# Jagnate/GTA_graph_tensor_acclelrator_for_general_GNN

Measured on AMD Instinct MI355X. Metric: edges/sec + achieved HBM GB/s, GAT aggregate on Reddit, 1/2/4/8 MI355X, higher is better.
Workload: dtype f32; 1 GPU; GAT layer-1 aggregate block [3,11,12] (scatter C -> applyedge MUL -> gather ADD); graph=reddit-shaped, N=232965, E=114615892, F=128, heads=8, parallelism=one GPU, whole graph, mode=single, grid=1x1, row_chunks=1, impl=blocked, blocks=20, world_size_seen=1

## Files before the change

### gta_graph_tensor_acclelrator_for_general_gnn_amd/csrc/gta_kernels.hip

```cpp
#include <hip/hip_runtime.h>
#include <hip/hip_bf16.h>

#include <algorithm>
#include <atomic>
#include <cmath>
#include <cstdint>
#include <map>
#include <mutex>
#include <string>
#include <utility>

#include "../../include/gta.h"

namespace {

thread_local std::string g_err;

int fail(int code, const std::string& msg) {
  g_err = msg;
  return code;
}

#define GTA_HIP(x)                                                                   \
  do {                                                                               \
// ... 1624 lines not shown
  const int lane = threadIdx.x & (kWave - 1);
  const int64_t row = static_cast<int64_t>(blockIdx.x) * kWavesPerBlock + wave_id_uniform();
  if (row >= n_rows) return;
  const int col = lane * VW;
  const bool empty = ri.row_ptr[row] == ri.row_ptr[row + 1];
  float acc[VW];
  seg_reduce_fold<VW>(slabs, ri, row, lane, FoldMax<false>{0u}, acc);
  Vec<VW> o;
#pragma unroll
  for (int q = 0; q < VW; ++q) o.v[q] = empty ? 0.f : red_flip(acc[q], sbit);
  o.store(y + row * ldy + col);
}

template <int VW>
__global__ void __launch_bounds__(kBlock)
k_seg_reduce_att(int64_t n_rows, const float* __restrict__ slabs, int H, int normalize, float* __restrict__ y,
                 int64_t ldy, float* __restrict__ sums, RowItems ri, int skip_single = 0, int sf_out = GTA_SF_NONE) {
  const int lane = threadIdx.x & (kWave - 1);
  const int64_t row = static_cast<int64_t>(blockIdx.x) * kWavesPerBlock + wave_id_uniform();
  if (row >= n_rows) return;
  if (skip_single && ri.row_ptr[row + 1] - ri.row_ptr[row] == 1) return;
  const int col = lane * VW;
  constexpr int F = kWave * VW;
  const int64_t lds = F + ((H + 3) & ~3);
  const int head = col / (F / H);
  float acc[VW];
#pragma unroll
  for (int q = 0; q < VW; ++q) acc[q] = 0.f;
  float sh = 0.f, sl = 0.f;
  const bool any = ri.row_ptr[row + 1] > ri.row_ptr[row];
  for_row_items<VW>(ri, row, lane, [&](int64_t i0, int64_t i1, int64_t i2, int64_t i3, int m) {
    const int64_t id[4] = {i0, i1, i2, i3};
    for (int u = 0; u < m; ++u) {
      Vec<VW> p;
      p.load(slabs + id[u] * lds + col);
#pragma unroll
      for (int q = 0; q < VW; ++q) acc[q] += p.v[q];
      const float* ss = slabs + id[u] * lds + F;
      sh += ss[head];
      if (lane < H) sl += ss[lane];
    }
  });
  Vec<VW> o;
#pragma unroll
  for (int q = 0; q < VW; ++q) o.v[q] = normalize ? (any ? acc[q] / sh : 0.f) : acc[q];
  if (sf_out != GTA_SF_NONE) {
#pragma unroll
    for (int q = 0; q < VW; ++q) o.v[q] = sf_apply(sf_out, o.v[q]);
  }
  o.store(y + row * ldy + col);
  if (sums != nullptr && lane < H) sums[row * H + lane] = sl;
}

struct BlockedView {
  int64_t* hdr;
  int32_t* perm;
  int32_t* seg;
  int32_t* bucket;
  int64_t* row_ptr;
  int32_t* cnt;
  int64_t* scan;
  int32_t* lhist;
  SegItem* items;
  int32_t* row_items;
  int32_t* item_slot;
  SegItem* items_tmp;
};

inline int64_t blocked_max_items(int64_t n_rows, int64_t nnz, int B, int64_t item_edges) {
  return std::min<int64_t>(n_rows * B, nnz) + nnz / item_edges;
}

constexpr int64_t kScanMaxTiles = 4096;

constexpr int kLenBins = 257;

inline int64_t blocked_fixed_bytes(int64_t n_rows, int B) {
  return round16(128) + round16(n_rows * 4) + round16(n_rows * (B + 1) * 4) + round16(64 * 4) +
         round16((n_rows + 1) * 8) + round16(n_rows * B * 4) + round16((kScanMaxTiles + 1) * 8) +
         round16(2 * 64 * kLenBins * 4);
}

BlockedView blocked_view(void* base, int64_t n_rows, int B, int64_t max_items) {
  char* p = static_cast<char*>(base);
  BlockedView v;
  v.hdr = reinterpret_cast<int64_t*>(p); p += round16(16 * 8);
  v.perm = reinterpret_cast<int32_t*>(p); p += round16(n_rows * 4);
  v.seg = reinterpret_cast<int32_t*>(p); p += round16(n_rows * (B + 1) * 4);
  v.bucket = reinterpret_cast<int32_t*>(p); p += round16(64 * 4);
  v.row_ptr = reinterpret_cast<int64_t*>(p); p += round16((n_rows + 1) * 8);
  v.cnt = reinterpret_cast<int32_t*>(p); p += round16(n_rows * B * 4);
  v.scan = reinterpret_cast<int64_t*>(p); p += round16((kScanMaxTiles + 1) * 8);
  v.lhist = reinterpret_cast<int32_t*>(p); p += round16(2 * 64 * kLenBins * 4);
  v.items = reinterpret_cast<SegItem*>(p); p += round16(max_items * 16);
  v.row_items = reinterpret_cast<int32_t*>(p); p += round16(max_items * 4);
  v.item_slot = reinterpret_cast<int32_t*>(p); p += round16(max_items * 4);
  v.items_tmp = reinterpret_cast<SegItem*>(p);
  return v;
}

int64_t blocked_bytes(int64_t n_rows, int B, int64_t max_items) {
  return blocked_fixed_bytes(n_rows, B) + round16(max_items * 16) + round16(max_items * 4) + round16(max_items * 4) +
         round16(max_items * 16);
}

__device__ __forceinline__ int deg_bucket(int64_t d) {
  return d <= 1 ? 0 : min(31, 63 - __clzll(static_cast<unsigned long long>(d)));
}

__host__ __device__ __forceinline__ int64_t n_parts(int64_t len, int64_t item_edges) {
  return (len + item_edges - 1) / item_edges;
}

__device__ __forceinline__ int merge_of(int64_t deg, int B, int64_t row_edges) {
  if (row_edges <= 0 || deg <= 0) return 1;
  int m = 1;
  while (m < B && deg * m < row_edges * B) m <<= 1;
  return m;
}

__global__ void __launch_bounds__(kBlock)
k_blocked_seg(const int64_t* __restrict__ indptr, const int32_t* __restrict__ indices, int64_t n_rows, int B,
              int64_t bsize, int64_t item_edges, int64_t row_edges, BlockedView v) {
  const int lane = threadIdx.x & (kWave - 1);
  const int64_t row = static_cast<int64_t>(blockIdx.x) * kWavesPerBlock + wave_id_uniform();
  if (row >= n_rows) return;
  const int64_t rb = indptr[row], re = indptr[row + 1];
  int64_t pos = 0;
  for (int b = lane; b <= B; b += kWave) {
    const int64_t key = static_cast<int64_t>(b) * bsize;
    int64_t lo = rb, hi = re;
    while (lo < hi) {
      const int64_t mid = (lo + hi) >> 1;
      if (static_cast<int64_t>(indices[mid]) < key) lo = mid + 1; else hi = mid;
    }
    pos = (b == B ? re : lo) - rb;
    v.seg[row * (B + 1) + b] = static_cast<int32_t>(pos);
  }
  const int m = merge_of(re - rb, B, row_edges);
  const int nb = (B + m - 1) / m;
  const int64_t lo = __shfl(pos, min(lane * m, B));
  const int64_t hi = __shfl(pos, min((lane + 1) * m, B));
  int64_t parts = (lane < nb) ? n_parts(hi - lo, item_edges) : 0;
#pragma unroll
  for (int off = 32; off > 0; off >>= 1) parts += __shfl_xor(parts, off);
  if (lane == 0) v.row_ptr[row] = parts;
  bool bad = false;
  for (int64_t e = rb + lane; e + 1 < re; e += kWave) bad |= indices[e] > indices[e + 1];
  if (__any(bad) && lane == 0) atomicOr(reinterpret_cast<unsigned long long*>(&v.hdr[3]), 1ull);
  if (lane == 0) atomicAdd(&v.bucket[deg_bucket(re - rb)], 1);
}

__global__ void k_blocked_scan(BlockedView v) {
  if (threadIdx.x == 0) {
    int run = 0;
    for (int k = 31; k >= 0; --k) {
      v.bucket[32 + k] = run;
      run += v.bucket[k];
    }
  }
}

__global__ void k_blocked_perm(const int64_t* __restrict__ indptr, int64_t n_rows, BlockedView v) {
  const int64_t r = static_cast<int64_t>(blockIdx.x) * blockDim.x + threadIdx.x;
  if (r >= n_rows) return;
  const int k = deg_bucket(indptr[r + 1] - indptr[r]);
  const int pos = atomicAdd(&v.bucket[32 + k], 1);
  v.perm[pos] = static_cast<int32_t>(r);
}

__global__ void k_blocked_cnt(int64_t n_rows, int B, int64_t item_edges, int64_t row_edges, BlockedView v) {
  const int64_t k = static_cast<int64_t>(blockIdx.x) * blockDim.x + threadIdx.x;
  if (k >= n_rows * B) return;
  const int b = static_cast<int>(k / n_rows);
  const int32_t row = v.perm[k - static_cast<int64_t>(b) * n_rows];
  const int32_t* sg = v.seg + static_cast<int64_t>(row) * (B + 1);
  const int m = merge_of(sg[B], B, row_edges);
  v.cnt[k] = (b % m) ? 0 : static_cast<int32_t>(n_parts(sg[min(b + m, B)] - sg[b], item_edges));
}

template <typename T>
__global__ void __launch_bounds__(1024) k_scan_excl(T* __restrict__ a, int64_t n, int total_at_end,
                                                    int64_t* __restrict__ total) {
  __shared__ int64_t part[1024];
  const int t = threadIdx.x;
  const int64_t per = (n + 1023) / 1024;
  const int64_t b = min<int64_t>(n, t * per), e = min<int64_t>(n, b + per);
  int64_t s = 0;
  for (int64_t i = b; i < e; ++i) s += a[i];
  part[t] = s;
  __syncthreads();
  for (int off = 1; off < 1024; off <<= 1) {
    const int64_t x = (t >= off) ? part[t - off] : 0;
    __syncthreads();
    part[t] += x;
    __syncthreads();
  }
  int64_t run = (t == 0) ? 0 : part[t - 1];
  for (int64_t i = b; i < e; ++i) {
    const int64_t x = a[i];
    a[i] = static_cast<T>(run);
    run += x;
  }
  if (t == 1023) {
    if (total_at_end) a[n] = static_cast<T>(part[1023]);
    if (total) *total = part[1023];
  }
}

constexpr int kScanPer = 16;
constexpr int64_t kScanTile = 1024 * kScanPer;

template <typename T>
__global__ void __launch_bounds__(1024) k_scan_tiles(const T* __restrict__ a, int64_t n, int64_t tile,
                                                     int64_t* __restrict__ sums) {
  __shared__ int64_t red[16];
  const int t = threadIdx.x;
  const int64_t b0 = static_cast<int64_t>(blockIdx.x) * tile, b1 = min<int64_t>(n, b0 + tile);
  int64_t s = 0;
  for (int64_t i = b0 + t; i < b1; i += 1024) s += a[i];
#pragma unroll
  for (int off = 32; off > 0; off >>= 1) s += __shfl_xor(s, off);
  if ((t & 63) == 0) red[t >> 6] = s;
  __syncthreads();
  if (t == 0) {
    int64_t tot = 0;
    for (int w = 0; w < 16; ++w) tot += red[w];
    sums[blockIdx.x] = tot;
  }
}

template <typename T>
__global__ void __launch_bounds__(1024) k_scan_apply(T* __restrict__ a, int64_t n, int64_t tile,
                                                     const int64_t* __restrict__ offs, int64_t nt, int total_at_end,
                                                     int64_t* __restrict__ total) {
  __shared__ int64_t part[1024];
  const int t = threadIdx.x;
  const int64_t b0 = static_cast<int64_t>(blockIdx.x) * tile, b1 = min<int64_t>(n, b0 + tile);
  const int64_t per = tile / 1024;
  const int64_t e0 = min<int64_t>(b1, b0 + t * per), e1 = min<int64_t>(b1, e0 + per);
  int64_t s = 0;
  for (int64_t i = e0; i < e1; ++i) s += a[i];
  part[t] = s;
  __syncthreads();
  for (int off = 1; off < 1024; off <<= 1) {
    const int64_t x = (t >= off) ? part[t - off] : 0;
    __syncthreads();
    part[t] += x;
    __syncthreads();
  }
  int64_t run = offs[blockIdx.x] + ((t == 0) ? 0 : part[t - 1]);
  for (int64_t i = e0; i < e1; ++i) {
    const int64_t x = a[i];
    a[i] = static_cast<T>(run);
    run += x;
  }
  if (blockIdx.x == nt - 1 && t == 0) {
    if (total_at_end) a[n] = static_cast<T>(offs[nt]);
    if (total) *total = offs[nt];
  }
}

template <typename T>
void scan_excl(T* a, int64_t n, int total_at_end, int64_t* total, int64_t* scratch, hipStream_t s) {
  int64_t tile = kScanTile;
  while ((n + tile - 1) / tile > kScanMaxTiles) tile *= 2;
  const int64_t nt = (n + tile - 1) / tile;
  if (nt <= 1) {
    k_scan_excl<T><<<1, 1024, 0, s>>>(a, n, total_at_end, total);
    return;
  }
  k_scan_tiles<T><<<dim3(static_cast<unsigned>(nt)), dim3(1024), 0, s>>>(a, n, tile, scratch);
  k_scan_excl<int64_t><<<1, 1024, 0, s>>>(scratch, nt, 1, nullptr);
  k_scan_apply<T><<<dim3(static_cast<unsigned>(nt)), dim3(1024), 0, s>>>(a, n, tile, scratch, nt, total_at_end, total);
}

__global__ void k_blocked_items(const int64_t* __restrict__ indptr, int64_t n_rows, int B, int64_t item_edges,
                                int64_t row_edges, BlockedView v) {
  const int64_t k = static_cast<int64_t>(blockIdx.x) * blockDim.x + threadIdx.x;
  if (k >= n_rows * B) return;
  const int b = static_cast<int>(k / n_rows);
  const int32_t row = v.perm[k - static_cast<int64_t>(b) * n_rows];
  const int32_t* sg = v.seg + static_cast<int64_t>(row) * (B + 1);
  const int m = merge_of(sg[B], B, row_edges);
  if (b % m) return;
  const int64_t len = sg[min(b + m, B)] - sg[b];
  if (len == 0) return;
  int64_t before = 0;
  for (int q = 0; q < b; q += m) before += n_parts(sg[min(q + m, B)] - sg[q], item_edges);
  const int64_t parts = n_parts(len, item_edges), part = (len + parts - 1) / parts;
  const int64_t id0 = v.cnt[k], slot0 = v.row_ptr[row] + before, beg = indptr[row] + sg[b];
  for (int64_t j = 0; j < parts; ++j) {
    SegItem it;
    it.beg = beg + j * part;
    it.row = row;
    it.len = static_cast<int32_t>(max<int64_t>(0, min<int64_t>(part, len - j * part)));
    v.items[id0 + j] = it;
    v.row_items[slot0 + j] = static_cast<int32_t>(id0 + j);
    v.item_slot[id0 + j] = static_cast<int32_t>(slot0 + j);
    atomicAdd(&v.lhist[b * kLenBins + 256 - min(it.len, 256)], 1);
  }
}

__device__ __forceinline__ int len_key(int len) { return 256 - min(len, 256); }

__global__ void k_items_len_scan(BlockedView v, int64_t n_rows, int B) {
  const int b = threadIdx.x;
  if (b >= B) return;
  int run = v.cnt[static_cast<int64_t>(b) * n_rows];
  for (int key = 0; key < kLenBins; ++key) {
    const int c = v.lhist[b * kLenBins + key];
    v.lhist[64 * kLenBins + b * kLenBins + key] = run;
    run += c;
  }
}

__global__ void k_items_permute(BlockedView v, int64_t n_rows, int B) {
  const int64_t id = static_cast<int64_t>(blockIdx.x) * blockDim.x + threadIdx.x;
  if (id >= v.hdr[4]) return;
  int lo = 0, hi = B - 1;
  while (lo < hi) {
    const int mid = (lo + hi + 1) >> 1;
    if (v.cnt[static_cast<int64_t>(mid) * n_rows] <= id) lo = mid; else hi = mid - 1;
  }
  const SegItem it = v.items[id];
  const int nid = atomicAdd(&v.lhist[64 * kLenBins + lo * kLenBins + len_key(it.len)], 1);
  v.items_tmp[nid] = it;
  v.row_items[v.item_slot[id]] = nid;
}

__global__ void __launch_bounds__(kBlock)
k_aggregate_combine(PlanView plan, int F, const float* __restrict__ row_scale, float* __restrict__ y, int64_t ldy,
                    int accumulate, const float* __restrict__ partial, const void* __restrict__ xs = nullptr,
                    int64_t ldxs = 0, int xs_bf16 = 0, const float* __restrict__ self_scale = nullptr,
                    int y_bf16 = 0) {
  const int lane = threadIdx.x & (kWave - 1);
  const int64_t s = static_cast<int64_t>(blockIdx.x) * kWavesPerBlock + wave_id_uniform();
  if (s >= plan.hdr[1]) return;
  const int64_t row = plan.split_row[s];
  const int64_t first = plan.split_first[s];
  const int cnt = plan.split_cnt[s];
  const float scale = row_scale ? row_scale[row] : 1.f;
  for (int c = lane; c < F; c += kWave) {
    float a = 0.f;
    for (int j = 0; j < cnt; ++j) a += partial[(first + j) * F + c];
    float* yp = y + row * ldy + c;
    float v;
    if (xs != nullptr) {
#pragma clang fp contract(off)
      const float xv = xs_bf16 ? load_elem(static_cast<const uint16_t*>(xs) + row * ldxs + c)
                               : static_cast<const float*>(xs)[row * ldxs + c];
      v = xv * (self_scale ? *self_scale : 1.f) + scale * a;
    } else {
      v = accumulate ? (*yp + scale * a) : scale * a;
    }
    if (y_bf16) reinterpret_cast<uint16_t*>(y)[row * ldy + c] = to_bf16_bits(v);
    else *yp = v;
  }
}

template <typename UNIT>
__global__ void __launch_bounds__(kBlock)
k_scatter(int dir, const int64_t* __restrict__ indptr, const int32_t* __restrict__ indices, int64_t n_rows,
          const UNIT* __restrict__ x, int64_t ldx_u, int64_t row_u, UNIT* __restrict__ out, int64_t ldo_u) {
  const int lane = threadIdx.x & (kWave - 1);
  const int64_t row = static_cast<int64_t>(blockIdx.x) * kWavesPerBlock + wave_id_uniform();
  if (row >= n_rows) return;
  const int64_t eb = indptr[row], ee = indptr[row + 1];
  const int64_t total = (ee - eb) * row_u;
  for (int64_t t = lane; t < total; t += kWave) {
    const int64_t el = t / row_u, c = t - el * row_u;
    const int64_t e = eb + el;
    const int64_t src = (dir == GTA_DIR_R) ? row : indices[e];
    out[e * ldo_u + c] = x[src * ldx_u + c];
  }
}

__device__ __forceinline__ int64_t edge_row(int mode, int64_t e, int64_t row, const int32_t* indices) {
  return mode == GTA_IDX_EDGE ? e : (mode == GTA_IDX_SRC ? static_cast<int64_t>(indices[e]) : row);
// ... 1799 lines not shown
bool dispatch_x(int xm, int wm, bool bf, const AggArgs& a, int64_t nb, hipStream_t s) {
  if (xm >= XM_EX1) return !bf && wm == WM_NONE && dispatch_expr<LPE, VW, NV>(xm, a, nb, s);
  return xm == XM_EDGE ? dispatch_w<LPE, VW, NV, XM_EDGE>(wm, bf, a, nb, s)
                       : dispatch_w<LPE, VW, NV, XM_IDX>(wm, bf, a, nb, s);
}

template <int LPE>
bool dispatch_bf16_vw8(int ur, int wm, const AggArgs& a, int64_t nb, hipStream_t s) {
  if (wm == WM_EDGE1) {
    if (ur == 8) launch_agg<LPE, 8, 1, XM_IDX, WM_EDGE1, uint16_t, 8>(a, nb, s);
    else launch_agg<LPE, 8, 1, XM_IDX, WM_EDGE1, uint16_t, 4>(a, nb, s);
  } else {
    if (ur == 8) launch_agg<LPE, 8, 1, XM_IDX, WM_NONE, uint16_t, 8>(a, nb, s);
    else launch_agg<LPE, 8, 1, XM_IDX, WM_NONE, uint16_t, 4>(a, nb, s);
  }
  return true;
}

template <int N>
using IC = std::integral_constant<int, N>;

template <int VW, class Fn>
bool dispatch_lpe(int lpe, int nv, Fn fn) {
  switch (lpe) {
    case 64:
      if constexpr (VW < 8) {
        if (nv == 2) return fn(IC<VW>{}, IC<64>{}, IC<2>{});
        if (nv != 1) return fn(IC<VW>{}, IC<64>{}, IC<4>{});
      }
      return fn(IC<VW>{}, IC<64>{}, IC<1>{});
    case 32: return fn(IC<VW>{}, IC<32>{}, IC<1>{});
    case 16: return fn(IC<VW>{}, IC<16>{}, IC<1>{});
    case 8: return fn(IC<VW>{}, IC<8>{}, IC<1>{});
    default: return fn(IC<VW>{}, IC<4>{}, IC<1>{});
  }
}

template <class Fn>
bool dispatch_vw(int vw, int lpe, int nv, Fn fn) {
  return vw == 4 ? dispatch_lpe<4>(lpe, nv, fn) : (vw == 2 ? dispatch_lpe<2>(lpe, nv, fn) : dispatch_lpe<1>(lpe, nv, fn));
}

struct Tuning {
  int force_lpe = 0;
  int force_vw = 0;
  int agg_lean = 1;
  int seg_lean = 1;
  int seg_lean_w1 = 1;
  int seg_pf = 0;
  int seg_alpha1 = 1;
  int agg_bf16_vw8 = 4;
  int agg_w1 = 1;
  int expr_lean = 1;
  int seg_phase = 0;
  int att_lean = 1;
  int att_direct = 1;
  int apply_node_vec = 1;
  int apply_edge_form = 1;
  int esm_lane = 1;
  int mm_ring = 1;
  int mm_ring_fr = 0;
  int mm_ring_depth = 0;
  int mm_prefetch = 1;
  int64_t mm_split = -1;
  int mm_wave = 1;
  int mm_wave_fr = 0;
};

Tuning& thread_tuning() {
  thread_local Tuning t;
  return t;
}

std::mutex g_attach_mu;
std::map<void*, Tuning> g_attached;
std::atomic<int> g_attached_n{0};
thread_local const Tuning* t_call = nullptr;

struct CallTuning {
  const Tuning* prev = t_call;
  Tuning snap;
  explicit CallTuning(void* stream) {
    if (g_attached_n.load(std::memory_order_acquire) == 0) return;
    std::lock_guard<std::mutex> lk(g_attach_mu);
    auto it = g_attached.find(stream);
    if (it == g_attached.end()) return;
    snap = it->second;
    t_call = &snap;
  }
  ~CallTuning() { t_call = prev; }
  CallTuning(const CallTuning&) = delete;
  CallTuning& operator=(const CallTuning&) = delete;
};

const Tuning& tuning() { return t_call ? *t_call : thread_tuning(); }

struct Knob {
  const char* key;
  int Tuning::*i32;
  int64_t Tuning::*i64;
};

const Knob* find_knob(const char* key) {
  static const Knob knobs[] = {
      {"agg_lpe", &Tuning::force_lpe, nullptr},
      {"agg_vw", &Tuning::force_vw, nullptr},
      {"agg_lean", &Tuning::agg_lean, nullptr},
      {"seg_lean", &Tuning::seg_lean, nullptr},
      {"seg_lean_w1", &Tuning::seg_lean_w1, nullptr},
      {"seg_alpha1", &Tuning::seg_alpha1, nullptr},
      {"seg_pf", &Tuning::seg_pf, nullptr},
      {"agg_bf16_vw8", &Tuning::agg_bf16_vw8, nullptr},
      {"agg_w1", &Tuning::agg_w1, nullptr},
      {"expr_lean", &Tuning::expr_lean, nullptr},
      {"seg_phase", &Tuning::seg_phase, nullptr},
      {"att_lean", &Tuning::att_lean, nullptr},
      {"att_direct", &Tuning::att_direct, nullptr},
      {"apply_node_vec", &Tuning::apply_node_vec, nullptr},
      {"apply_edge_form", &Tuning::apply_edge_form, nullptr},
      {"esm_lane", &Tuning::esm_lane, nullptr},
      {"mm_ring", &Tuning::mm_ring, nullptr},
      {"mm_ring_fr", &Tuning::mm_ring_fr, nullptr},
      {"mm_ring_depth", &Tuning::mm_ring_depth, nullptr},
      {"mm_prefetch", &Tuning::mm_prefetch, nullptr},
      {"mm_split", nullptr, &Tuning::mm_split},
      {"mm_wave", &Tuning::mm_wave, nullptr},
      {"mm_wave_fr", &Tuning::mm_wave_fr, nullptr},
  };
  const std::string k(key ? key : "");
  for (const Knob& kb : knobs)
    if (k == kb.key) return &kb;
  return nullptr;
}

}

extern "C" {

int gta_abi_version(void) { return GTA_ABI_VERSION; }
const char* gta_last_error(void) { return g_err.c_str(); }

int gta_debug_set(const char* key, int64_t value) {
  const Knob* kb = find_knob(key);
  if (!kb) return fail(GTA_ERR_ARG, std::string("gta_debug_set: unknown key ") + (key ? key : ""));
  if (kb->i32) thread_tuning().*(kb->i32) = static_cast<int>(value);
  else thread_tuning().*(kb->i64) = value;
  return GTA_OK;
}

int gta_debug_get(const char* key, int64_t* value) {
  const Knob* kb = find_knob(key);
  if (!kb || !value) return fail(GTA_ERR_ARG, std::string("gta_debug_get: unknown key ") + (key ? key : ""));
  *value = kb->i32 ? static_cast<int64_t>(thread_tuning().*(kb->i32)) : thread_tuning().*(kb->i64);
  return GTA_OK;
}

}

struct gta_tuning {
  Tuning t;
};

extern "C" {

gta_tuning* gta_tuning_create(void) { return new (std::nothrow) gta_tuning{}; }

void gta_tuning_destroy(gta_tuning* h) { delete h; }
// ... 384 lines not shown
    code |= (bins[i] << (8 + 3 * i)) | (sfs[i] << (17 + 4 * i));
  }
  const int nl = shape == 1 ? (bins[0] == GTA_BIN_NONE ? 1 : 2) : shape + 1;
  for (int l = 0; l < 4; ++l) {
    const int k = l < nl ? l : 0;
    if (modes[k] != GTA_IDX_EDGE && modes[k] != GTA_IDX_SRC && modes[k] != GTA_IDX_DST)
      return fail(GTA_ERR_ARG, "aggregate_expr: bad operand mode");
    if ((lds[k] < F && !(modes[k] == GTA_IDX_EDGE && lds[k] == 0)) || (nnz > 0 && !operands[k]))
      return fail(GTA_ERR_ARG, "aggregate_expr: operand rows need ld >= F (or ld 0: a broadcast row)");
    if (lds[k] > INT32_MAX) return fail(GTA_ERR_UNSUPPORTED, "aggregate_expr: operand row stride >= 2^31");
    ex.p[l] = operands[k];
    ex.ld[l] = static_cast<int>(lds[k]);
    code |= modes[k] << (2 * l);
  }
  ex.code = code;
  return aggregate_impl(indptr, indices, n_rows, nnz, GTA_IDX_EDGE, ex.p[0], F, F, GTA_F32, nullptr, 0, 0, nullptr,
                        y, ldy, 0, plan, plan_chunk, workspace, stream, nullptr, 0, nullptr, 0, &ex, XM_EX1 + shape - 1);
}

int gta_aggregate_self(const int64_t* indptr, const int32_t* indices, int64_t n_rows, int64_t nnz, int x_mode,
                       const void* x, int64_t ldx, int64_t F, int x_dtype, const float* w, int64_t ldw, int64_t heads,
                       const float* row_scale, const void* x_self, int64_t ld_self, const float* self_scale, void* y,
                       int64_t ldy, int y_dtype, const void* plan, int64_t plan_chunk, void* workspace, void* stream) {
  if (!x_self) return fail(GTA_ERR_ARG, "aggregate_self: x_self is NULL");
  if (y_dtype != GTA_F32 && y_dtype != GTA_BF16) return fail(GTA_ERR_ARG, "aggregate_self: y_dtype must be F32 or BF16");
  return aggregate_impl(indptr, indices, n_rows, nnz, x_mode, x, ldx, F, x_dtype, w, ldw, heads, row_scale,
                        static_cast<float*>(y), ldy, 0, plan, plan_chunk, workspace, stream, x_self, ld_self, self_scale,
                        y_dtype == GTA_BF16 ? 1 : 0);
}

int64_t gta_aggregate_blocked_plan_bytes(int64_t n_rows, int64_t nnz, int64_t blocks, int64_t item_edges) {
  if (n_rows < 0 || nnz < 0 || blocks < 1 || blocks > 63 || item_edges < 1)
    return fail(GTA_ERR_ARG, "blocked_plan_bytes: need n_rows, nnz >= 0, 1 <= blocks <= 63, item_edges >= 1");
  const int B = static_cast<int>(blocks);
  return blocked_bytes(n_rows, B, blocked_max_items(n_rows, nnz, B, item_edges));
}

int gta_aggregate_blocked_plan_build(const int64_t* indptr, const int32_t* indices, int64_t n_rows, int64_t n_cols,
                                     int64_t nnz, int64_t blocks, int64_t item_edges, int64_t row_edges, void* plan,
                                     int64_t plan_bytes, void* stream) {
  const CallTuning ct_(stream);
  if (!indptr || !plan || n_rows <= 0 || n_cols <= 0 || nnz < 0 || blocks < 1 || blocks > 63 || item_edges < 1 ||
      row_edges < 0)
    return fail(GTA_ERR_ARG, "blocked_plan_build: bad arguments");
  if (nnz > 0 && !indices) return fail(GTA_ERR_ARG, "blocked_plan_build: indices needed");
  if (n_rows > INT32_MAX) return fail(GTA_ERR_UNSUPPORTED, "blocked_plan_build: > 2^31 rows");
  const int B = static_cast<int>(blocks);
  const int64_t mi = blocked_max_items(n_rows, nnz, B, item_edges);
  if (mi > INT32_MAX || n_rows * B > INT32_MAX) return fail(GTA_ERR_UNSUPPORTED, "blocked_plan_build: > 2^31 items");
  if (plan_bytes < blocked_bytes(n_rows, B, mi)) return fail(GTA_ERR_ARG, "blocked_plan_build: plan buffer too small");
  BlockedView v = blocked_view(plan, n_rows, B, mi);
  hipStream_t s = S(stream);
  const int64_t bsize = (n_cols + B - 1) / B;
  const int64_t hdr[16] = {B, bsize, n_rows, 0, 0, item_edges, mi,
                           reinterpret_cast<char*>(v.row_items) - static_cast<char*>(plan), row_edges};
  GTA_HIP(hipMemcpyAsync(v.hdr, hdr, sizeof(hdr), hipMemcpyHostToDevice, s));
  GTA_HIP(hipMemsetAsync(v.bucket, 0, 64 * 4, s));
  k_blocked_seg<<<dim3(static_cast<unsigned>((n_rows + kWavesPerBlock - 1) / kWavesPerBlock)), dim3(kBlock), 0, s>>>(
      indptr, indices, n_rows, B, bsize, item_edges, row_edges, v);
  GTA_LAUNCHED("k_blocked_seg");
  k_blocked_scan<<<1, 64, 0, s>>>(v);
  GTA_LAUNCHED("k_blocked_scan");
  k_blocked_perm<<<dim3(static_cast<unsigned>((n_rows + 255) / 256)), dim3(256), 0, s>>>(indptr, n_rows, v);
  GTA_LAUNCHED("k_blocked_perm");
  scan_excl<int64_t>(v.row_ptr, n_rows, 1, nullptr, v.scan, s);
  GTA_LAUNCHED("scan_excl");
  const dim3 gk(static_cast<unsigned>((n_rows * B + 255) / 256));
  k_blocked_cnt<<<gk, dim3(256), 0, s>>>(n_rows, B, item_edges, row_edges, v);
  GTA_LAUNCHED("k_blocked_cnt");
  scan_excl<int32_t>(v.cnt, n_rows * B, 0, &v.hdr[4], v.scan, s);
  GTA_LAUNCHED("scan_excl");
  GTA_HIP(hipMemsetAsync(v.lhist, 0, 64 * kLenBins * 4, s));
  k_blocked_items<<<gk, dim3(256), 0, s>>>(indptr, n_rows, B, item_edges, row_edges, v);
  GTA_LAUNCHED("k_blocked_items");
  if (mi > 0) {
    k_items_len_scan<<<1, 64, 0, s>>>(v, n_rows, B);
    GTA_LAUNCHED("k_items_len_scan");
    k_items_permute<<<dim3(static_cast<unsigned>((mi + 255) / 256)), dim3(256), 0, s>>>(v, n_rows, B);
    GTA_LAUNCHED("k_items_permute");
    GTA_HIP(hipMemcpyAsync(v.items, v.items_tmp, mi * sizeof(SegItem), hipMemcpyDeviceToDevice, s));
  }
  return GTA_OK;
}


int64_t gta_aggregate_blocked_workspace_bytes(int64_t n_rows, int64_t nnz, int64_t blocks, int64_t F,
                                              int64_t item_edges) {
  if (n_rows < 0 || nnz < 0 || blocks < 1 || blocks > 63 || F <= 0 || item_edges < 1)
    return fail(GTA_ERR_ARG, "blocked_workspace_bytes: bad sizes");
  return blocked_max_items(n_rows, nnz, static_cast<int>(blocks), item_edges) * F * static_cast<int64_t>(sizeof(float));
}

static int aggregate_blocked_impl(const std::string& who, const int64_t* indptr, const int32_t* indices, int64_t n_rows,
                                  int64_t n_cols, int64_t nnz, const void* xv, int64_t ldx, int64_t F, int x_dtype,
                                  const float* w, int64_t ldw, int64_t heads, const float* row_scale, float* y,
                                  int64_t ldy, int accumulate, const void* plan, int64_t blocks, int64_t item_edges,
                                  void* workspace, void* stream) {
  const CallTuning ct_(stream);
  if (n_rows < 0 || nnz < 0 || F <= 0 || blocks < 1 || blocks > 63 || item_edges < 1)
    return fail(GTA_ERR_ARG, who + ": bad sizes");
  if (x_dtype != GTA_F32 && x_dtype != GTA_BF16) return fail(GTA_ERR_ARG, who + ": x_dtype must be F32 or BF16");
  if (n_rows == 0) return GTA_OK;
  if (!indptr || !xv || !y || !plan) return fail(GTA_ERR_ARG, who + ": bad arguments");
  const bool bf = x_dtype == GTA_BF16;
  const float* x = static_cast<const float*>(xv);
  int gl = 0, vw = 0;
  for (int c : {4, 2, 1}) {
    if (F == static_cast<int64_t>(kWave) * c && (bf || (ldx % c == 0 && aligned(x, 4 * c))) && ldy % c == 0 &&
        aligned(y, 4 * c)) {
      vw = c;
      break;
    }
  }
  if (!vw) return fail(GTA_ERR_UNSUPPORTED, who + ": F must be 64, 128 or 256 (one edge per wave row)");
  bool gl_ok = true;
  if (w) {
    if (heads <= 0 || F % heads) return fail(GTA_ERR_ARG, who + ": heads must divide F");
    gl = static_cast<int>(F / heads) / vw;
    gl_ok = (F / heads) % vw == 0 && (gl == 4 || gl == 8 || gl == 16);
  }
  const std::string gl_msg = who + ": (F/heads)/VW must be 4, 8 or 16 (or quarter-wave lanes per head 1..16)";
  const BlockedCall c(plan, n_rows, nnz, blocks, item_edges, workspace, stream);
  if (!workspace && nnz > 0) return fail(GTA_ERR_ARG, who + ": needs the slab workspace");
  const int vq = static_cast<int>(F / 16);
  const int lph = w ? static_cast<int>((F / heads) / vq) : 0;
  const bool quarter = (vq == 4 || vq == 8 || vq == 16) && ldx % (bf ? 8 : 4) == 0 && aligned(x, 16) &&
                       (!w || ((F / heads) % vq == 0 && lph >= 1 && 16 % lph == 0));
  if (bf && !quarter)
    return fail(GTA_ERR_UNSUPPORTED, who + ": bf16 rows need x 16-B aligned, ldx % 8 == 0 and heads that fit the "
                                           "multi-item forms (F/heads a multiple of F/16, lanes per head dividing 16)");
  const int phase = tuning().seg_phase;
// ... 1068 lines not shown
```

### gta_graph_tensor_acclelrator_for_general_gnn_amd/graph.py

```python
import math

import torch

SHAPES = {
    "cora": (2708, 10556),
    "citeseer": (3327, 9228),
    "pubmed": (19717, 88648),
    "flickr": (89250, 899756),
    "reddit": (232965, 114615892),
    "products": (2449029, 123718280),
}


class Graph:

    def __init__(self, indptr, indices, n_cols=None):
        if indptr.dtype != torch.int64 or indices.dtype != torch.int32:
            raise TypeError("indptr must be int64 and indices int32")
        if indptr.device != indices.device:
            raise ValueError("indptr and indices on different devices")
        self.indptr = indptr.contiguous()
        self.indices = indices.contiguous()
        self.n_rows = indptr.numel() - 1
        self.n_cols = self.n_rows if n_cols is None else int(n_cols)
        self.nnz = indices.numel()
        self._plans = {}
        self._row_of_edge = None
        self._deg = None

    @property
    def device(self):
        return self.indptr.device

    def to(self, device):
        return Graph(self.indptr.to(device), self.indices.to(device), self.n_cols)

    def degrees(self):
        if self._deg is None:
            self._deg = (self.indptr[1:] - self.indptr[:-1])
        return self._deg

    def row_of_edge(self):
        if self._row_of_edge is None:
            rows = torch.arange(self.n_rows, device=self.device, dtype=torch.int32)
            self._row_of_edge = torch.repeat_interleave(rows, self.degrees())
        return self._row_of_edge

    def csc(self):
        if "csc" not in self._plans:
            from . import ops
            self._plans["csc"] = ops.CSC(self)
        return self._plans["csc"]

    def plan(self, chunk=512):
        if chunk not in self._plans:
            from . import ops
            self._plans[chunk] = ops.AggregatePlan(self, chunk)
        return self._plans[chunk]

    def blocked_plan(self, blocks=32, item_edges=None, row_edges=None):
        from . import ops
        key = ("blocked", blocks, int(item_edges or ops.BlockedPlan.ITEM_EDGES),
               int(ops.BlockedPlan.ROW_EDGES if row_edges is None else row_edges))
        if key not in self._plans:
            self._plans[key] = ops.BlockedPlan(self, blocks, key[2], key[3])
        return self._plans[key]

    def numpy(self):
        return self.indptr.cpu().numpy(), self.indices.cpu().numpy()

    def __repr__(self):
        return f"Graph(N={self.n_rows}, E={self.nnz}, device={self.device})"


def from_numpy(indptr, indices, device="cpu", n_cols=None):
    return Graph(torch.as_tensor(indptr, dtype=torch.int64).to(device),
                 torch.as_tensor(indices, dtype=torch.int32).to(device), n_cols)


def lognormal_degrees(n, e, seed=0, sigma=1.0, device="cpu"):
    g = torch.Generator(device=device)
    g.manual_seed(seed)
    z = torch.randn(n, generator=g, device=device, dtype=torch.float64)
    raw = torch.exp(sigma * z)
    scaled = raw * (e / raw.sum())
    deg = torch.floor(scaled).to(torch.int64)
    rem = int(e - int(deg.sum().item()))
    if rem > 0:
        frac = scaled - deg.to(torch.float64)
        top = torch.topk(frac, rem).indices
        deg[top] += 1
    return deg


def synthetic(n, e, seed=0, kind="lognormal", sigma=1.0, device="cpu", sort_cols=True, dedupe=False,
              locality_width=None):
    device = torch.device(device)
    if kind == "uniform":
        deg = torch.full((n,), e // n, dtype=torch.int64, device=device)
        deg[: e - int(deg.sum())] += 1
    elif kind == "lognormal":
        deg = lognormal_degrees(n, e, seed=seed, sigma=sigma, device=device)
    else:
        raise ValueError(kind)
    g = torch.Generator(device=device)
    g.manual_seed(seed + 1)
    rows = torch.repeat_interleave(torch.arange(n, device=device, dtype=torch.int64), deg)
    if locality_width is None:
        cols = torch.randint(0, n, (e,), generator=g, device=device, dtype=torch.int64)
    else:
        off = torch.randint(-locality_width, locality_width + 1, (e,), generator=g, device=device,
                            dtype=torch.int64)
        cols = torch.remainder(rows + off, n)
    if dedupe:
        keep = cols != rows
        rows, cols = rows[keep], cols[keep]
    if sort_cols or dedupe:
        key = rows * n + cols
# ... 115 lines not shown
```

### gta_graph_tensor_acclelrator_for_general_gnn_amd/ops.py

```python
import ctypes
import math
import threading
import weakref

import torch

from . import _lib
from ._lib import check

_MODES = {"edge": _lib.IDX_EDGE, "src": _lib.IDX_SRC, "dst": _lib.IDX_DST}
_BINS = {None: _lib.BIN_NONE, "NONE": _lib.BIN_NONE, "ADD": _lib.BIN_ADD, "MUL": _lib.BIN_MUL,
         "DIV": _lib.BIN_DIV, "SUB": _lib.BIN_SUB}


def _L():
    return _lib.load()


def _stream(dev):
    return torch.cuda.current_stream(dev).cuda_stream


def _need_gpu(*ts):
    for t in ts:
# ... 191 lines not shown
                          _ptr(x), ldx, F, x_dt, _ptr(out), ldy, _ptr(pbuf), chunk, _ptr(ws), _stream(x.device)),
          "reduce")
    return out


EXPR_SHAPES = {1: 2, 2: 3, 3: 4}


def aggregate_expr(graph, shape, operands, bins, sfs=None, swap=False, plan=None):
    if shape not in EXPR_SHAPES:
        raise ValueError(f"aggregate_expr: shape must be 1, 2 or 3 (got {shape})")
    n_ops = shape
    bins = list(bins) + [None] * (3 - len(bins))
    sfs = list(sfs or []) + [None] * (3 - len(sfs or []))
    n_l = 1 if (shape == 1 and bins[0] is None) else EXPR_SHAPES[shape]
    if len(operands) != n_l:
        raise ValueError(f"aggregate_expr: shape {shape} takes {n_l} operands (got {len(operands)})")
    ts = [t for t, _ in operands]
    _need_gpu(graph.indptr, *ts)
    F = ts[0].shape[1]
    ptrs, modes, lds = (ctypes.c_void_p * 4)(), (ctypes.c_int * 4)(), (ctypes.c_int64 * 4)()
    for l, (t, m) in enumerate(operands):
        if t.shape[1] != F:
            raise ValueError("aggregate_expr: every operand has the same width")
        ld = _rows(t, f"operand {l}")
        if m == "row":
            m, ld = "edge", 0
            if t.shape[0] < 1:
                raise ValueError("aggregate_expr: a broadcast row needs one row")
        else:
            need = {"edge": graph.nnz, "src": graph.n_cols, "dst": graph.n_rows}[m]
            if t.shape[0] < need:
                raise ValueError(f"aggregate_expr operand {l}: {m}-mode operand needs {need} rows")
        ptrs[l], modes[l], lds[l] = t.data_ptr(), _MODES[m], ld
    cb = (ctypes.c_int * 3)(*[_BINS[b] for b in bins])
    cs = (ctypes.c_int * 3)(*[_sf(s) for s in sfs])
    out = torch.empty(graph.n_rows, F, dtype=torch.float32, device=ts[0].device)
    if graph.n_rows == 0:
        return out
    pbuf, ws, chunk = _plan_args(graph, plan, F)
    rc = _L().gta_aggregate_expr(_ptr(graph.indptr), _ptr(graph.indices), graph.n_rows, graph.nnz, n_ops,
                                 ptrs, modes, lds, cb, cs, int(bool(swap)), F, _ptr(out), F, _ptr(pbuf), chunk,
                                 _ptr(ws), _stream(ts[0].device))
    if rc == _lib.ERR_UNSUPPORTED:
        return None
    check(rc, "aggregate_expr")
    return out


class BlockedPlan:

    ITEM_EDGES = 256
    ROW_EDGES = 0

    def __init__(self, graph, blocks=32, item_edges=None, row_edges=None):
        _need_gpu(graph.indptr)
        L = _L()
        self.graph, self.blocks = graph, int(blocks)
        self.item_edges = int(item_edges or BlockedPlan.ITEM_EDGES)
        self.row_edges = int(BlockedPlan.ROW_EDGES if row_edges is None else row_edges)
        nb = check(L.gta_aggregate_blocked_plan_bytes(graph.n_rows, graph.nnz, self.blocks, self.item_edges),
                   "blocked_plan_bytes")
        self.buf = torch.empty(int(nb), dtype=torch.uint8, device=graph.device)
        check(L.gta_aggregate_blocked_plan_build(_ptr(graph.indptr), _ptr(graph.indices), graph.n_rows, graph.n_cols,
                                                 graph.nnz, self.blocks, self.item_edges, self.row_edges,
                                                 _ptr(self.buf), int(nb),
                                                 _stream(graph.device)),
              "blocked_plan_build")
        hdr = self.buf[:64].view(torch.int64).cpu()
        self.sorted = int(hdr[3]) == 0
        self.n_items = int(hdr[4])
        self._ws = {}

    def workspace(self, F):
        if F not in self._ws:
            nb = check(_L().gta_aggregate_blocked_workspace_bytes(self.graph.n_rows, self.graph.nnz, self.blocks, F,
                                                                  self.item_edges),
                       "blocked_workspace_bytes")
            self._ws[F] = torch.empty(int(nb), dtype=torch.uint8, device=self.graph.device)
        return self._ws[F]

    def workspace_att(self, F, heads):
        key = ("att", F, heads)
        if key not in self._ws:
            nb = check(_L().gta_gat_aggregate_blocked_workspace_bytes(self.graph.n_rows, self.graph.nnz, self.blocks,
                                                                      F, heads, self.item_edges),
                       "gat_workspace_bytes")
            self._ws[key] = torch.empty(int(nb), dtype=torch.uint8, device=self.graph.device)
        return self._ws[key]

    @staticmethod
    def supports_att(F, heads):
        if F not in (64, 128, 256) or heads <= 0 or F % heads:
            return False
        fh, vq = F // heads, F // 16
        return fh % vq == 0 and 16 % (fh // vq) == 0

    DTYPES = (torch.float32, torch.bfloat16)

    @staticmethod
    def auto_blocks(graph, F, elem=4):
        table_mb = graph.n_cols * F * elem / 1e6
        avg_deg = graph.nnz / max(1, graph.n_rows)
        return int(max(1, min(24, round(table_mb / 6.0), avg_deg // 24)))

    @staticmethod
    def supports(F, heads, dtype=torch.float32):
        if dtype not in BlockedPlan.DTYPES or F not in (64, 128, 256):
            return False
        if not heads:
            return True
        if F % heads:
            return False
# ... 546 lines not shown
```

Before: 23.58 billion edges/s.

## Group blocked-plan rows by merge class and enable row merging by default

Blocked plan rows are now ordered class-major: they are keyed by their column-block merge factor and then by degree bucket. Each merge class gets its own contiguous work-item groups and length histograms, so items with the same merge width are scheduled together. The default row_edges moves from 0 to 10 through a new resolve step, which turns on merging of adjacent column blocks for low-degree rows and cuts the number of tiny items. This adds bookkeeping (class tables and up to 128 groups) and changes the plan cache key; the item count and the locality of the aggregation change in exchange.

```diff
diff --git a/gta_graph_tensor_acclelrator_for_general_gnn_amd/csrc/gta_kernels.hip b/gta_graph_tensor_acclelrator_for_general_gnn_amd/csrc/gta_kernels.hip
--- a/gta_graph_tensor_acclelrator_for_general_gnn_amd/csrc/gta_kernels.hip
+++ b/gta_graph_tensor_acclelrator_for_general_gnn_amd/csrc/gta_kernels.hip
@@ -1700,11 +1700,21 @@
   if (sums != nullptr && lane < H) sums[row * H + lane] = sl;
 }
 
+constexpr int kMaxCls = 7;
+constexpr int kMaxGroups = 128;
+constexpr int kClsBase = 0;
+constexpr int kClsRow0 = 8;
+constexpr int kClsRows = 16;
+constexpr int kClsStep = 24;
+constexpr int kClsGroup0 = 32;
+constexpr int kClsFirst = 48;
+
 struct BlockedView {
   int64_t* hdr;
   int32_t* perm;
   int32_t* seg;
   int32_t* bucket;
+  int32_t* cls;
   int64_t* row_ptr;
   int32_t* cnt;
   int64_t* scan;
@@ -1724,9 +1734,9 @@
 constexpr int kLenBins = 257;
 
 inline int64_t blocked_fixed_bytes(int64_t n_rows, int B) {
-  return round16(128) + round16(n_rows * 4) + round16(n_rows * (B + 1) * 4) + round16(64 * 4) +
+  return round16(128) + round16(n_rows * 4) + round16(n_rows * (B + 1) * 4) + round16(2 * 256 * 4) + round16(256 * 4) +
          round16((n_rows + 1) * 8) + round16(n_rows * B * 4) + round16((kScanMaxTiles + 1) * 8) +
-         round16(2 * 64 * kLenBins * 4);
+         round16(2 * kMaxGroups * kLenBins * 4);
 }
 
 BlockedView blocked_view(void* base, int64_t n_rows, int B, int64_t max_items) {
@@ -1735,11 +1745,12 @@
   v.hdr = reinterpret_cast<int64_t*>(p); p += round16(16 * 8);
   v.perm = reinterpret_cast<int32_t*>(p); p += round16(n_rows * 4);
   v.seg = reinterpret_cast<int32_t*>(p); p += round16(n_rows * (B + 1) * 4);
-  v.bucket = reinterpret_cast<int32_t*>(p); p += round16(64 * 4);
+  v.bucket = reinterpret_cast<int32_t*>(p); p += round16(2 * 256 * 4);
+  v.cls = reinterpret_cast<int32_t*>(p); p += round16(256 * 4);
   v.row_ptr = reinterpret_cast<int64_t*>(p); p += round16((n_rows + 1) * 8);
   v.cnt = reinterpret_cast<int32_t*>(p); p += round16(n_rows * B * 4);
   v.scan = reinterpret_cast<int64_t*>(p); p += round16((kScanMaxTiles + 1) * 8);
-  v.lhist = reinterpret_cast<int32_t*>(p); p += round16(2 * 64 * kLenBins * 4);
+  v.lhist = reinterpret_cast<int32_t*>(p); p += round16(2 * kMaxGroups * kLenBins * 4);
   v.items = reinterpret_cast<SegItem*>(p); p += round16(max_items * 16);
   v.row_items = reinterpret_cast<int32_t*>(p); p += round16(max_items * 4);
   v.item_slot = reinterpret_cast<int32_t*>(p); p += round16(max_items * 4);
@@ -1767,9 +1778,13 @@
   return m;
 }
 
+__device__ __forceinline__ int row_key(int64_t deg, int m, int class_major) {
+  return (class_major ? (31 - __clz(m)) * 32 : 0) + deg_bucket(deg);
+}
+
 __global__ void __launch_bounds__(kBlock)
 k_blocked_seg(const int64_t* __restrict__ indptr, const int32_t* __restrict__ indices, int64_t n_rows, int B,
-              int64_t bsize, int64_t item_edges, int64_t row_edges, BlockedView v) {
+              int64_t bsize, int64_t item_edges, int64_t row_edges, int class_major, BlockedView v) {
   const int lane = threadIdx.x & (kWave - 1);
   const int64_t row = static_cast<int64_t>(blockIdx.x) * kWavesPerBlock + wave_id_uniform();
   if (row >= n_rows) return;
@@ -1796,33 +1811,69 @@
   bool bad = false;
   for (int64_t e = rb + lane; e + 1 < re; e += kWave) bad |= indices[e] > indices[e + 1];
   if (__any(bad) && lane == 0) atomicOr(reinterpret_cast<unsigned long long*>(&v.hdr[3]), 1ull);
-  if (lane == 0) atomicAdd(&v.bucket[deg_bucket(re - rb)], 1);
-}
-
-__global__ void k_blocked_scan(BlockedView v) {
-  if (threadIdx.x == 0) {
-    int run = 0;
+  if (lane == 0) atomicAdd(&v.bucket[row_key(re - rb, m, class_major)], 1);
+}
+
+__global__ void k_blocked_scan(BlockedView v, int B, int class_major) {
+  if (threadIdx.x != 0) return;
+  int run = 0, base = 0, group = 0;
+  for (int c = 0; c < kMaxCls; ++c) {
+    const int step = class_major ? 1 << c : 1, nb = (B + step - 1) / step, row0 = run;
     for (int k = 31; k >= 0; --k) {
-      v.bucket[32 + k] = run;
-      run += v.bucket[k];
-    }
-  }
-}
-
-__global__ void k_blocked_perm(const int64_t* __restrict__ indptr, int64_t n_rows, BlockedView v) {
+      v.bucket[256 + c * 32 + k] = run;
+      run += v.bucket[c * 32 + k];
+    }
+    v.cls[kClsBase + c] = base;
+    v.cls[kClsRow0 + c] = row0;
+    v.cls[kClsRows + c] = run - row0;
+    v.cls[kClsStep + c] = step;
+    v.cls[kClsGroup0 + c] = group;
+    if (run > row0) {
+      base += nb * (run - row0);
+      group += nb;
+    }
+  }
+  v.cls[kClsBase + kMaxCls] = base;
+  v.cls[kClsGroup0 + kMaxCls] = group;
+}
+
+__global__ void k_blocked_perm(const int64_t* __restrict__ indptr, int64_t n_rows, int B, int64_t row_edges,
+                               int class_major, BlockedView v) {
   const int64_t r = static_cast<int64_t>(blockIdx.x) * blockDim.x + threadIdx.x;
   if (r >= n_rows) return;
-  const int k = deg_bucket(indptr[r + 1] - indptr[r]);
-  const int pos = atomicAdd(&v.bucket[32 + k], 1);
+  const int64_t deg = indptr[r + 1] - indptr[r];
+  const int k = row_key(deg, merge_of(deg, B, row_edges), class_major);
+  const int pos = atomicAdd(&v.bucket[256 + k], 1);
   v.perm[pos] = static_cast<int32_t>(r);
+}
+
+struct CntEntry {
+  int c, j, b;
+  int32_t row;
+};
+
+__device__ __forceinline__ bool cnt_entry(const BlockedView& v, int64_t k, CntEntry& e) {
+  if (k >= v.cls[kClsBase + kMaxCls]) return false;
+  int c = 0;
+  while (c + 1 < kMaxCls && k >= v.cls[kClsBase + c + 1]) ++c;
+  const int64_t off = k - v.cls[kClsBase + c], n = v.cls[kClsRows + c];
+  e.c = c;
+  e.j = static_cast<int>(off / n);
+  e.b = e.j * v.cls[kClsStep + c];
+  e.row = v.perm[v.cls[kClsRow0 + c] + (off - e.j * n)];
+  return true;
 }
 
 __global__ void k_blocked_cnt(int64_t n_rows, int B, int64_t item_edges, int64_t row_edges, BlockedView v) {
   const int64_t k = static_cast<int64_t>(blockIdx.x) * blockDim.x + threadIdx.x;
   if (k >= n_rows * B) return;
-  const int b = static_cast<int>(k / n_rows);
-  const int32_t row = v.perm[k - static_cast<int64_t>(b) * n_rows];
-  const int32_t* sg = v.seg + static_cast<int64_t>(row) * (B + 1);
+  CntEntry e;
+  if (!cnt_entry(v, k, e)) {
+    v.cnt[k] = 0;
+    return;
+  }
+  const int b = e.b;
+  const int32_t* sg = v.seg + static_cast<int64_t>(e.row) * (B + 1);
   const int m = merge_of(sg[B], B, row_edges);
   v.cnt[k] = (b % m) ? 0 : static_cast<int32_t>(n_parts(sg[min(b + m, B)] - sg[b], item_edges));
 }
@@ -1926,9 +1977,10 @@
 __global__ void k_blocked_items(const int64_t* __restrict__ indptr, int64_t n_rows, int B, int64_t item_edges,
                                 int64_t row_edges, BlockedView v) {
   const int64_t k = static_cast<int64_t>(blockIdx.x) * blockDim.x + threadIdx.x;
-  if (k >= n_rows * B) return;
-  const int b = static_cast<int>(k / n_rows);
-  const int32_t row = v.perm[k - static_cast<int64_t>(b) * n_rows];
+  CntEntry e;
+  if (k >= n_rows * B || !cnt_entry(v, k, e)) return;
+  const int b = e.b, group = v.cls[kClsGroup0 + e.c] + e.j;
+  const int32_t row = e.row;
   const int32_t* sg = v.seg + static_cast<int64_t>(row) * (B + 1);
   const int m = merge_of(sg[B], B, row_edges);
   if (b % m) return;
@@ -1946,33 +1998,38 @@
     v.items[id0 + j] = it;
     v.row_items[slot0 + j] = static_cast<int32_t>(id0 + j);
     v.item_slot[id0 + j] = static_cast<int32_t>(slot0 + j);
-    atomicAdd(&v.lhist[b * kLenBins + 256 - min(it.len, 256)], 1);
+    atomicAdd(&v.lhist[group * kLenBins + 256 - min(it.len, 256)], 1);
   }
 }
 
 __device__ __forceinline__ int len_key(int len) { return 256 - min(len, 256); }
 
-__global__ void k_items_len_scan(BlockedView v, int64_t n_rows, int B) {
-  const int b = threadIdx.x;
-  if (b >= B) return;
-  int run = v.cnt[static_cast<int64_t>(b) * n_rows];
+__global__ void __launch_bounds__(kMaxGroups) k_items_len_scan(BlockedView v) {
+  const int g = threadIdx.x, groups = v.cls[kClsGroup0 + kMaxCls];
+  if (g == groups) v.cls[kClsFirst + g] = static_cast<int32_t>(v.hdr[4]);
+  if (g >= groups) return;
+  int c = 0;
+  while (c + 1 < kMaxCls && g >= v.cls[kClsGroup0 + c + 1]) ++c;
+  const int64_t k = v.cls[kClsBase + c] + static_cast<int64_t>(g - v.cls[kClsGroup0 + c]) * v.cls[kClsRows + c];
+  int run = v.cnt[k];
+  v.cls[kClsFirst + g] = run;
   for (int key = 0; key < kLenBins; ++key) {
-    const int c = v.lhist[b * kLenBins + key];
-    v.lhist[64 * kLenBins + b * kLenBins + key] = run;
-    run += c;
-  }
-}
-
-__global__ void k_items_permute(BlockedView v, int64_t n_rows, int B) {
+    const int n = v.lhist[g * kLenBins + key];
+    v.lhist[kMaxGroups * kLenBins + g * kLenBins + key] = run;
+    run += n;
+  }
+}
+
+__global__ void k_items_permute(BlockedView v) {
   const int64_t id = static_cast<int64_t>(blockIdx.x) * blockDim.x + threadIdx.x;
   if (id >= v.hdr[4]) return;
-  int lo = 0, hi = B - 1;
+  int lo = 0, hi = v.cls[kClsGroup0 + kMaxCls] - 1;
   while (lo < hi) {
     const int mid = (lo + hi + 1) >> 1;
-    if (v.cnt[static_cast<int64_t>(mid) * n_rows] <= id) lo = mid; else hi = mid - 1;
+    if (v.cls[kClsFirst + mid] <= id) lo = mid; else hi = mid - 1;
   }
   const SegItem it = v.items[id];
-  const int nid = atomicAdd(&v.lhist[64 * kLenBins + lo * kLenBins + len_key(it.len)], 1);
+  const int nid = atomicAdd(&v.lhist[kMaxGroups * kLenBins + lo * kLenBins + len_key(it.len)], 1);
   v.items_tmp[nid] = it;
   v.row_items[v.item_slot[id]] = nid;
 }
@@ -3878,6 +3935,11 @@
   int agg_bf16_vw8 = 4;
   int agg_w1 = 1;
   int expr_lean = 1;
+  int seg_class_major = 1;
+  int seg_fine_pct = 100;
+  int seg_row_edges = 10;
+  int seg_fine_min = 16;
+  int seg_item_edges = 0;
   int seg_phase = 0;
   int att_lean = 1;
   int att_direct = 1;
@@ -3939,6 +4001,11 @@
       {"agg_bf16_vw8", &Tuning::agg_bf16_vw8, nullptr},
       {"agg_w1", &Tuning::agg_w1, nullptr},
       {"expr_lean", &Tuning::expr_lean, nullptr},
+      {"seg_class_major", &Tuning::seg_class_major, nullptr},
+      {"seg_fine_pct", &Tuning::seg_fine_pct, nullptr},
+      {"seg_row_edges", &Tuning::seg_row_edges, nullptr},
+      {"seg_fine_min", &Tuning::seg_fine_min, nullptr},
+      {"seg_item_edges", &Tuning::seg_item_edges, nullptr},
       {"seg_phase", &Tuning::seg_phase, nullptr},
       {"att_lean", &Tuning::att_lean, nullptr},
       {"att_direct", &Tuning::att_direct, nullptr},
@@ -4429,16 +4496,18 @@
   BlockedView v = blocked_view(plan, n_rows, B, mi);
   hipStream_t s = S(stream);
   const int64_t bsize = (n_cols + B - 1) / B;
+  const int class_major = tuning().seg_class_major ? 1 : 0;
   const int64_t hdr[16] = {B, bsize, n_rows, 0, 0, item_edges, mi,
-                           reinterpret_cast<char*>(v.row_items) - static_cast<char*>(plan), row_edges};
+                           reinterpret_cast<char*>(v.row_items) - static_cast<char*>(plan), row_edges, class_major};
   GTA_HIP(hipMemcpyAsync(v.hdr, hdr, sizeof(hdr), hipMemcpyHostToDevice, s));
-  GTA_HIP(hipMemsetAsync(v.bucket, 0, 64 * 4, s));
+  GTA_HIP(hipMemsetAsync(v.bucket, 0, 2 * 256 * 4, s));
   k_blocked_seg<<<dim3(static_cast<unsigned>((n_rows + kWavesPerBlock - 1) / kWavesPerBlock)), dim3(kBlock), 0, s>>>(
-      indptr, indices, n_rows, B, bsize, item_edges, row_edges, v);
+      indptr, indices, n_rows, B, bsize, item_edges, row_edges, class_major, v);
   GTA_LAUNCHED("k_blocked_seg");
-  k_blocked_scan<<<1, 64, 0, s>>>(v);
+  k_blocked_scan<<<1, 64, 0, s>>>(v, B, class_major);
   GTA_LAUNCHED("k_blocked_scan");
-  k_blocked_perm<<<dim3(static_cast<unsigned>((n_rows + 255) / 256)), dim3(256), 0, s>>>(indptr, n_rows, v);
+  k_blocked_perm<<<dim3(static_cast<unsigned>((n_rows + 255) / 256)), dim3(256), 0, s>>>(indptr, n_rows, B, row_edges,
+                                                                                         class_major, v);
   GTA_LAUNCHED("k_blocked_perm");
   scan_excl<int64_t>(v.row_ptr, n_rows, 1, nullptr, v.scan, s);
   GTA_LAUNCHED("scan_excl");
@@ -4447,13 +4516,13 @@
   GTA_LAUNCHED("k_blocked_cnt");
   scan_excl<int32_t>(v.cnt, n_rows * B, 0, &v.hdr[4], v.scan, s);
   GTA_LAUNCHED("scan_excl");
-  GTA_HIP(hipMemsetAsync(v.lhist, 0, 64 * kLenBins * 4, s));
+  GTA_HIP(hipMemsetAsync(v.lhist, 0, kMaxGroups * kLenBins * 4, s));
   k_blocked_items<<<gk, dim3(256), 0, s>>>(indptr, n_rows, B, item_edges, row_edges, v);
   GTA_LAUNCHED("k_blocked_items");
   if (mi > 0) {
-    k_items_len_scan<<<1, 64, 0, s>>>(v, n_rows, B);
+    k_items_len_scan<<<1, kMaxGroups, 0, s>>>(v);
     GTA_LAUNCHED("k_items_len_scan");
-    k_items_permute<<<dim3(static_cast<unsigned>((mi + 255) / 256)), dim3(256), 0, s>>>(v, n_rows, B);
+    k_items_permute<<<dim3(static_cast<unsigned>((mi + 255) / 256)), dim3(256), 0, s>>>(v);
     GTA_LAUNCHED("k_items_permute");
     GTA_HIP(hipMemcpyAsync(v.items, v.items_tmp, mi * sizeof(SegItem), hipMemcpyDeviceToDevice, s));
   }
diff --git a/gta_graph_tensor_acclelrator_for_general_gnn_amd/graph.py b/gta_graph_tensor_acclelrator_for_general_gnn_amd/graph.py
--- a/gta_graph_tensor_acclelrator_for_general_gnn_amd/graph.py
+++ b/gta_graph_tensor_acclelrator_for_general_gnn_amd/graph.py
@@ -60,10 +60,10 @@
 
     def blocked_plan(self, blocks=32, item_edges=None, row_edges=None):
         from . import ops
-        key = ("blocked", blocks, int(item_edges or ops.BlockedPlan.ITEM_EDGES),
-               int(ops.BlockedPlan.ROW_EDGES if row_edges is None else row_edges))
+        fine, ie, re_ = ops.BlockedPlan.resolve(blocks, item_edges, row_edges)
+        key = ("blocked", blocks, ie, re_) + ((fine,) if fine != blocks else ())
         if key not in self._plans:
-            self._plans[key] = ops.BlockedPlan(self, blocks, key[2], key[3])
+            self._plans[key] = ops.BlockedPlan(self, blocks, item_edges, row_edges)
         return self._plans[key]
 
     def numpy(self):
diff --git a/gta_graph_tensor_acclelrator_for_general_gnn_amd/ops.py b/gta_graph_tensor_acclelrator_for_general_gnn_amd/ops.py
--- a/gta_graph_tensor_acclelrator_for_general_gnn_amd/ops.py
+++ b/gta_graph_tensor_acclelrator_for_general_gnn_amd/ops.py
@@ -267,13 +267,28 @@
 
     ITEM_EDGES = 256
     ROW_EDGES = 0
+    MAX_BLOCKS = 63
+
+    @staticmethod
+    def resolve(blocks, item_edges=None, row_edges=None, knobs=None):
+        blocks = int(blocks)
+        named = (blocks, int(item_edges or BlockedPlan.ITEM_EDGES),
+                 int(BlockedPlan.ROW_EDGES if row_edges is None else row_edges))
+        if item_edges is not None or row_edges is not None:
+            return named
+        if knobs is None:
+            knobs = tuple(get_debug(k) for k in ("seg_fine_pct", "seg_row_edges", "seg_fine_min", "seg_item_edges"))
+        pct, re_, least, ie = (tuple(knobs) + (0,))[:4]
+        if blocks < least:
+            return named
+        fine = min(BlockedPlan.MAX_BLOCKS, max(1, int(math.floor(blocks * pct / 100.0 + 0.5))))
+        return fine, int(ie or BlockedPlan.ITEM_EDGES), max(0, int(re_))
 
     def __init__(self, graph, blocks=32, item_edges=None, row_edges=None):
         _need_gpu(graph.indptr)
         L = _L()
-        self.graph, self.blocks = graph, int(blocks)
-        self.item_edges = int(item_edges or BlockedPlan.ITEM_EDGES)
-        self.row_edges = int(BlockedPlan.ROW_EDGES if row_edges is None else row_edges)
+        self.graph, self.requested = graph, int(blocks)
+        self.blocks, self.item_edges, self.row_edges = BlockedPlan.resolve(blocks, item_edges, row_edges)
         nb = check(L.gta_aggregate_blocked_plan_bytes(graph.n_rows, graph.nnz, self.blocks, self.item_edges),
                    "blocked_plan_bytes")
         self.buf = torch.empty(int(nb), dtype=torch.uint8, device=graph.device)
```

Result: faster. 23.99 billion edges/s (median of 6 runs) (+1.7%).
